# nz0001na/MorphGANformer

Measured on AMD Instinct MI355X. Metric: latent-projection iters/sec @1024^2, k=17 latents, higher is better.
Workload: dtype f32; 1 GPU; configs[1]: single 1024x1024 face per GPU, Wing+LPIPS(squeeze)+MSE literal-mode projection step, noise_mode=random, seeded synthetic weights/targets/landmarks; k=17, z_dim=32, targets_per_gpu=1, parallelism=pair-sharded x1, graph_replay=True, loss_generator_overlap=True, steps_per_forward=32

## Files before the change

include/mgf.h:

```cpp
#ifndef MGF_H_
#define MGF_H_

#include <stdint.h>

#ifdef __cplusplus
extern "C" {
#endif

typedef void* mgf_stream_t;

enum { MGF_OK = 0, MGF_EINVAL = -1, MGF_EUNSUPPORTED = -2, MGF_ELAUNCH = -3, MGF_ETOOBIG = -4 };
enum { MGF_F32 = 0, MGF_F64 = 1, MGF_F16 = 2 };
enum { MGF_FILTER_SEPARABLE = 2 };
enum { MGF_FILTER_LARGE = 4 };
enum { MGF_ACT_LINEAR = 1, MGF_ACT_RELU = 2, MGF_ACT_LRELU = 3, MGF_ACT_TANH = 4, MGF_ACT_SIGMOID = 5,
       MGF_ACT_ELU = 6, MGF_ACT_SELU = 7, MGF_ACT_SOFTPLUS = 8, MGF_ACT_SWISH = 9,
       MGF_ACT_RELU_POST = 10 };

const char* mgf_last_error(void);
int mgf_version(void);
int mgf_device_ok(void);

int mgf_bias_act(void* y, const void* x, const void* b, const void* xref, const void* yref, const void* dy,
                 int dtype, int64_t numel, int64_t step_b, int64_t size_b,
// ... 66 lines not shown
                                  const float* rgb_w, const float* rgb_bias, int32_t n, int32_t cin, int32_t h, int32_t w, int32_t cout,
                                  int32_t out_scale_stride, int32_t rgb_channels, mgf_stream_t stream);
int mgf_conv3x3_winograd2_f32(float* y, const float* x, const float* u, const float* in_scale, const float* out_scale, int32_t n,
                              int32_t cin, int32_t h, int32_t w, int32_t cout, int32_t out_scale_stride, const mgf_epilogue* ep,
                              mgf_stream_t stream);
int mgf_conv3x3_winograd3_f32(float* y, const float* x, const float* u, const float* in_scale, const float* out_scale, int32_t n,
                              int32_t cin, int32_t h, int32_t w, int32_t cout, int32_t out_scale_stride, const mgf_epilogue* ep,
                              mgf_stream_t stream);
int mgf_conv3x3_winograd3_slice_f32(float* y, const float* x, const float* u, const float* in_scale, const float* out_scale, int32_t n,
                                    int32_t cin, int32_t h, int32_t w, int32_t cout, int32_t out_scale_stride, int64_t y_batch,
                                    int32_t y_choff, const mgf_epilogue* ep, mgf_stream_t stream);
int mgf_conv1x1_f32(float* y, const float* x, const float* w, const float* in_scale, int32_t n, int32_t cin, int32_t hw, int32_t cout,
                    int32_t cout_pad, int64_t y_batch, int32_t y_choff, const mgf_epilogue* ep, mgf_stream_t stream);
int mgf_conv1x1_force_shape(int32_t channel_blocks);

int mgf_conv3x3s2_few_inputs_f32(float* y, const float* x, const float* w, const float* bias, int32_t n, int32_t cin, int32_t in_h,
                                 int32_t in_w, int32_t cout, int32_t relu, mgf_stream_t stream);
int mgf_tconv3x3s2_few_outputs_f32(float* y, const float* x, const float* wp, int32_t n, int32_t cin, int32_t h, int32_t w, int32_t cout,
                                   int32_t cout_pad, int32_t pitch, int64_t y_plane, int64_t y_batch, mgf_stream_t stream);
int mgf_conv3x3_winograd3_up2res_f32(float* y, const float* x, const float* u, const float* in_scale, const float* out_scale,
                                     const float* residual_low, int32_t n, int32_t cin, int32_t h, int32_t w, int32_t cout,
                                     int32_t out_scale_stride, const mgf_epilogue* ep, mgf_stream_t stream);
int mgf_winograd3_force_shape(int32_t shape);
int mgf_conv3x3_winograd3_rgb_f32(float* rgb_out, const float* x, const float* u, const float* in_scale, const float* out_scale,
                                  const float* rgb_w, const float* rgb_bias, int32_t n, int32_t cin, int32_t h, int32_t w, int32_t cout,
                                  int32_t out_scale_stride, int32_t rgb_channels, mgf_stream_t stream);
int mgf_conv3x3_winograd_f32(float* y, const float* x, const float* u, const float* in_scale, const float* out_scale, int32_t n,
                             int32_t cin, int32_t h, int32_t w, int32_t cout, int32_t out_scale_stride, const mgf_epilogue* ep,
                             mgf_stream_t stream);

int mgf_tconv3x3s2_border_f32(float* t, const float* x, const float* wp, const float* in_scale, const float* out_scale, int32_t n,
                              int32_t cin, int32_t h, int32_t w, int32_t cout, int32_t cout_pad, int64_t t_pitch, int64_t t_plane,
                              int64_t t_batch, int64_t out_scale_stride, mgf_stream_t stream);

int mgf_pack_conv_weights(float* wp, float* wsq, const float* w, int32_t cout, int32_t cin, int32_t kh, int32_t kw,
                          int32_t cout_pad, float gain, int32_t flip, mgf_stream_t stream);

typedef struct mgf_style_job {
    const float* aff_w;
    const float* aff_b;
    const float* wsq;
    float* s;
    float* d;
    int32_t cin, cout;
    int32_t w_offset;
    float aff_gain, style_gain;
} mgf_style_job;
int mgf_demod_f32(float* d, const float* s, const float* wsq, int32_t n, int32_t cin, int32_t cout, mgf_stream_t stream);
int mgf_demod_bwd_f32(float* ds, const float* dd, const float* d, const float* s, const float* wsq, int32_t n, int32_t cin, int32_t cout,
                      mgf_stream_t stream);
int mgf_style_demod(const mgf_style_job* job, const float* ws, int64_t ws_stride_n, int32_t n, int32_t wdim, mgf_stream_t stream);
int mgf_style_demod_multi(const mgf_style_job* jobs_dev, int32_t njobs, const float* ws, int64_t ws_stride_n,
                          int32_t n, int32_t wdim, int32_t max_cin, mgf_stream_t stream);

int mgf_duplex_attention(float* y, const float* x, const float* wqc, const float* spos, const float* vwb,
                         int32_t n, int32_t c, int32_t f, int32_t t,
                         const mgf_epilogue* ep, int32_t ep_w, float* probs, int32_t* argmax, mgf_stream_t stream);

int mgf_att_map_upsample_f32(float* out, const float* probs, int32_t n, int32_t side, int32_t t, int32_t out_res, int32_t layer,
                             int32_t n_layers, mgf_stream_t stream);

typedef struct mgf_attn_job {
    const float* wmv;
    const float* bmv;
    float* vwb;
    int32_t c;
// ... 188 lines not shown
```

morphganformer_amd/_lib.py:

```python
from __future__ import annotations

import ctypes as C
import os

import torch

HERE = os.path.dirname(os.path.abspath(__file__))
LIB_PATH = os.environ.get("MGF_LIB_PATH") or os.path.join(HERE, "libmgf_hip.so")

MGF_F32, MGF_F64, MGF_F16 = 0, 1, 2
ACT_IDS = {"linear": 1, "relu": 2, "lrelu": 3, "tanh": 4, "sigmoid": 5, "elu": 6, "selu": 7, "softplus": 8, "swish": 9,
           "relu_post": 10}
MAX_TAPS = 9

i32, i64, f32, f64, vp = C.c_int32, C.c_int64, C.c_float, C.c_double, C.c_void_p


class Epilogue(C.Structure):
    _fields_ = [("bias", vp), ("noise", vp), ("noise_strength", vp), ("noise_n", i32), ("act", i32), ("alpha", f32),
                ("gain", f32), ("residual", vp)]


class ConvDesc(C.Structure):
    _fields_ = [("n", i32), ("cin", i32), ("in_h", i32), ("in_w", i32), ("cout", i32), ("cout_pad", i32),
# ... 11 lines not shown
class StyleJob(C.Structure):
    _fields_ = [("aff_w", vp), ("aff_b", vp), ("wsq", vp), ("s", vp), ("d", vp), ("cin", i32), ("cout", i32),
                ("w_offset", i32), ("aff_gain", f32), ("style_gain", f32)]


class AttnJob(C.Structure):
    _fields_ = [("wmv", vp), ("bmv", vp), ("vwb", vp), ("c", i32), ("w_offset", i32)]


class StyleBwdJob(C.Structure):
    _fields_ = [("aff_w", vp), ("wsq", vp), ("s", vp), ("d", vp), ("ds_part", vp), ("dc_part", vp), ("cin", i32), ("cout", i32),
                ("s_chunks", i32), ("d_chunks", i32), ("aff_gain", f32), ("style_gain", f32)]


class AttnGradJob(C.Structure):
    _fields_ = [("dg", vp), ("probs", vp), ("dc", vp), ("cpre", vp), ("part", vp), ("dvwb", vp), ("dc_part", vp), ("c", i32), ("f", i32),
                ("slices", i32), ("nchunk", i32), ("blk_grad", i32), ("blk_dot", i32), ("blk_red", i32), ("pad_", i32)]


class AttnBwdJob(C.Structure):
    _fields_ = [("wmv", vp), ("dvwb", vp), ("c", i32), ("pad_", i32)]


_SIGS = {
    "mgf_last_error": (C.c_char_p, []),
    "mgf_version": (C.c_int, []),
    "mgf_device_ok": (C.c_int, []),
    "mgf_bias_act": (C.c_int, [vp, vp, vp, vp, vp, vp, C.c_int, i64, i64, i64, C.c_int, C.c_int, f32, f32, f32, vp]),
    "mgf_upfirdn2d": (C.c_int, [vp, vp, vp, C.c_int, i32, i32, i32, i32, i64, i64, i64, i64, i32, i32, i64, i64, i64, i64,
                                i32, i32, i32, i32, i32, i32, i32, i32, i32, i32, i32, f32, C.POINTER(Epilogue), vp]),
    "mgf_conv_taps_f32": (C.c_int, [vp, vp, vp, vp, vp, C.POINTER(ConvDesc), C.POINTER(Epilogue), vp]),
    "mgf_conv_taps_bf16x3_f32": (C.c_int, [vp, vp, vp, vp, vp, C.POINTER(ConvDesc), C.POINTER(Epilogue), vp]),
    "mgf_tconv3x3s2_border_f32": (C.c_int, [vp, vp, vp, vp, vp, i32, i32, i32, i32, i32, i32, i64, i64, i64, i64, vp]),
    "mgf_winograd_weights_f32": (C.c_int, [vp, vp, i32, i32, f32, vp]),
    "mgf_conv3x3_winograd_f32": (C.c_int, [vp, vp, vp, vp, vp, i32, i32, i32, i32, i32, i32, C.POINTER(Epilogue), vp]),
    "mgf_winograd2_weights_f32": (C.c_int, [vp, vp, i32, i32, f32, vp]),
    "mgf_conv3x3_winograd2_f32": (C.c_int, [vp, vp, vp, vp, vp, i32, i32, i32, i32, i32, i32, C.POINTER(Epilogue), vp]),
    "mgf_conv3x3_winograd2_rgb_f32": (C.c_int, [vp, vp, vp, vp, vp, vp, vp, i32, i32, i32, i32, i32, i32, i32, vp]),
    "mgf_conv3x3_winograd3_f32": (C.c_int, [vp, vp, vp, vp, vp, i32, i32, i32, i32, i32, i32, C.POINTER(Epilogue), vp]),
    "mgf_conv1x1_f32": (C.c_int, [vp, vp, vp, vp, i32, i32, i32, i32, i32, i64, i32, C.POINTER(Epilogue), vp]),
    "mgf_conv3x3s2_few_inputs_f32": (C.c_int, [vp, vp, vp, vp, i32, i32, i32, i32, i32, i32, vp]),
    "mgf_tconv3x3s2_few_outputs_f32": (C.c_int, [vp, vp, vp, i32, i32, i32, i32, i32, i32, i32, i64, i64, vp]),
    "mgf_conv1x1_force_shape": (C.c_int, [i32]),
    "mgf_conv3x3_winograd3_slice_f32": (C.c_int, [vp, vp, vp, vp, vp, i32, i32, i32, i32, i32, i32, i64, i32, C.POINTER(Epilogue), vp]),
    "mgf_conv3x3_winograd3_up2res_f32": (C.c_int, [vp, vp, vp, vp, vp, vp, i32, i32, i32, i32, i32, i32, C.POINTER(Epilogue), vp]),
    "mgf_winograd3_force_shape": (C.c_int, [i32]),
    "mgf_conv3x3_winograd3_rgb_f32": (C.c_int, [vp, vp, vp, vp, vp, vp, vp, i32, i32, i32, i32, i32, i32, i32, vp]),
    "mgf_conv3x3_winograd2_slice_f32": (C.c_int, [vp, vp, vp, vp, vp, i32, i32, i32, i32, i32, i32, i64, i32, C.POINTER(Epilogue), vp]),
    "mgf_pack_conv_weights": (C.c_int, [vp, vp, vp, i32, i32, i32, i32, i32, f32, i32, vp]),
    "mgf_conv_profile_begin": (C.c_int, []),
    "mgf_conv_profile_end": (C.c_int, [C.POINTER(ConvProfRec), i32]),
    "mgf_demod_f32": (C.c_int, [vp, vp, vp, i32, i32, i32, vp]),
    "mgf_demod_bwd_f32": (C.c_int, [vp, vp, vp, vp, vp, i32, i32, i32, vp]),
    "mgf_style_demod": (C.c_int, [C.POINTER(StyleJob), vp, i64, i32, i32, vp]),
    "mgf_style_demod_multi": (C.c_int, [vp, i32, vp, i64, i32, i32, i32, vp]),
    "mgf_duplex_attention": (C.c_int, [vp, vp, vp, vp, vp, i32, i32, i32, i32, C.POINTER(Epilogue), i32, vp, vp, vp]),
    "mgf_att_map_upsample_f32": (C.c_int, [vp, vp, i32, i32, i32, i32, i32, i32, vp]),
    "mgf_attn_values": (C.c_int, [C.POINTER(AttnJob), vp, i64, i64, i32, i32, i32, vp]),
    "mgf_attn_values_multi": (C.c_int, [vp, i32, vp, i64, i64, i32, i32, i32, vp]),
    "mgf_randn_f32": (C.c_int, [vp, i64, C.c_uint64, vp, vp]),
    "mgf_rgb_weights_f32": (C.c_int, [vp, vp, vp, i32, i32, i32, vp]),
    "mgf_torgb_compose_weights_f32": (C.c_int, [vp, vp, vp, vp, vp, vp, i32, i32, i32, i32, vp]),
    "mgf_conv3x3_few_outputs_f32": (C.c_int, [vp, vp, vp, vp, i32, i32, i32, i32, i32, vp]),
    "mgf_mapping_param_floats": (i64, [i32, i32, i32]),
    "mgf_mapping_forward": (C.c_int, [vp, vp, vp, i32, i32, i32, i32, i32, vp]),
    "mgf_reduce_scratch_floats": (i64, []),
# ... 134 lines not shown
```

morphganformer_amd/build.py:

```python
from __future__ import annotations

import glob
import hashlib
import os
import subprocess
import sys

HERE = os.path.dirname(os.path.abspath(__file__))
ROOT = os.path.dirname(HERE)
CSRC = os.path.join(HERE, "csrc")
OBJ = os.path.join(CSRC, "_obj")
LIB = os.path.join(HERE, "libmgf_hip.so")
SOURCES = ["capi.cpp", "bias_act.hip", "upfirdn2d.hip", "conv_taps.hip", "latent_prep.hip", "attention.hip", "losses.hip", "lpips_stem.hip",
           "embed.hip", "backward.hip", "wino.hip", "wino3.hip", "pointwise.hip", "narrow_conv.hip", "warp.hip", "lbp.hip", "mdf.hip"]
HEADERS = [os.path.join(CSRC, "mgf_common.h"), os.path.join(ROOT, "include", "mgf.h")]
HIPCC = os.environ.get("HIPCC", "/opt/rocm/bin/hipcc")
FLAGS = ["--offload-arch=gfx950", "-O3", "-fPIC", "-std=c++17", "-ffp-contract=on", "-Wno-unused-result", "-x", "hip"]
LINK_FLAGS = ["--offload-arch=gfx950", "-shared", "-fPIC"]

_compiler_id = None


def compiler_id() -> str:
    global _compiler_id
    if _compiler_id is None:
        _compiler_id = subprocess.run([HIPCC, "--version"], stdout=subprocess.PIPE, stderr=subprocess.STDOUT, check=True).stdout.decode()
    return _compiler_id


def object_key(src_path: str, flags) -> str:
    h = hashlib.sha256()
    h.update(compiler_id().encode())
    h.update("\0".join(flags).encode())
    for p in [src_path] + HEADERS:
        with open(p, "rb") as f:
            h.update(b"\0" + os.path.basename(p).encode() + b"\0" + f.read())
    return h.hexdigest()[:16]


def _compile_all(obj_dir, flags_for, verbose, force, prune=True):
    os.makedirs(obj_dir, exist_ok=True)
    objs, todo = [], []
    for src in SOURCES:
        sp = os.path.join(CSRC, src)
        flags = flags_for(src)
        op = os.path.join(obj_dir, f"{src}.{object_key(sp, flags)}.o")
        objs.append(op)
# ... 95 lines not shown
```

morphganformer_amd/conv.py:

```python
from __future__ import annotations

import ctypes as C
import os
from dataclasses import dataclass

import torch

from . import _lib


def round_up(v: int, m: int) -> int:
    return (v + m - 1) // m * m


def profile_begin():
    _lib.check(_lib.lib().mgf_conv_profile_begin(), "conv_profile_begin")


def profile_end(max_recs=4096):
    recs = (_lib.ConvProfRec * max_recs)()
    n = _lib.lib().mgf_conv_profile_end(recs, max_recs)
    if n < 0:
        _lib.check(n, "conv_profile_end")
    return [(recs[i].kernel.decode(), recs[i].flops, recs[i].seconds, recs[i].ksplit, recs[i].bytes) for i in range(min(n, max_recs))]
# ... 341 lines not shown
    return round_up(2 * w + 1, align)


def conv3x3s2_few_inputs(x, w, bias=None, relu=False, out=None):
    _lib.require_gpu(x, w, bias, out)
    cout, cin = w.shape[:2]
    assert tuple(w.shape[2:]) == (3, 3) and cin <= 4 and w.is_contiguous() and w.dtype == torch.float32
    assert x.dtype == torch.float32 and x.is_contiguous() and x.shape[1] == cin
    n, _, h, wd = x.shape
    oh, ow = (h - 3) // 2 + 1, (wd - 3) // 2 + 1
    if out is None:
        out = torch.empty([n, cout, oh, ow], dtype=torch.float32, device=x.device)
    assert out.is_contiguous() and tuple(out.shape) == (n, cout, oh, ow)
    rc = _lib.lib().mgf_conv3x3s2_few_inputs_f32(out.data_ptr(), x.data_ptr(), w.data_ptr(), _lib.ptr(bias), n, cin, h, wd, cout, int(relu),
                                                 _lib.stream_ptr())
    _lib.check(rc, "conv3x3s2_few_inputs")
    return out


def conv3x3_few_outputs(x, w, bias=None, out=None):
    _lib.require_gpu(x, w, bias, out)
    n, cin, h, wd = x.shape
    cout = w.shape[1]
    assert x.dtype == torch.float32 and x.is_contiguous() and w.dtype == torch.float32 and w.is_contiguous()
    assert tuple(w.shape) == (n, cout, cin, 3, 3) and cout <= 4
    if out is None:
        out = torch.empty([n, cout, h, wd], dtype=torch.float32, device=x.device)
    assert out.is_contiguous() and tuple(out.shape) == (n, cout, h, wd)
    _lib.check(_lib.lib().mgf_conv3x3_few_outputs_f32(out.data_ptr(), x.data_ptr(), w.data_ptr(), _lib.ptr(bias), n, cin, h, wd, cout,
                                                      _lib.stream_ptr()), "conv3x3_few_outputs")
    return out


def tconv3x3s2_forward(x, pc: PackedConv, in_scale=None, out_scale=None, out=None, bf=None):
    _lib.require_gpu(x, pc.wp, in_scale, out_scale, out)
    assert pc.kh == 3 and pc.kw == 3 and x.dtype == torch.float32 and x.is_contiguous()
    n, cin, h, w = x.shape
    oh, ow = 2 * h + 1, 2 * w + 1
    if out is None:
        out = torch.empty([n, pc.cout, oh, tconv_pitch(w)], dtype=torch.float32, device=x.device)
    pitch = out.shape[3]
    assert out.is_contiguous() and tuple(out.shape) == (n, pc.cout, oh, pitch) and pitch >= ow and pitch % 4 == 0
    if NARROW_CONV and pc.cout <= 4 and in_scale is None and out_scale is None:
        rc = _lib.lib().mgf_tconv3x3s2_few_outputs_f32(out.data_ptr(), x.data_ptr(), pc.wp.data_ptr(), n, cin, h, w, pc.cout, pc.cout_pad,
                                                       pitch, oh * pitch, pc.cout * oh * pitch, _lib.stream_ptr())
        _lib.check(rc, "tconv3x3s2_few_outputs")
        return out[:, :, :, :ow]
    split = SPLIT_TCONV_BORDER and min(h, w) >= (TCONV_SPLIT_MIN if n >= 4 else max(TCONV_SPLIT_MIN, 128))
    use_bf = bf is not None and split and w % 32 == 0 and cin % 16 == 0
    os_stride = 0 if out_scale is None else out_scale.stride(0) if out_scale.ndim == 2 else 0
    d = _desc(n, cin, h, w, pc.cout, pc.cout_pad, h if split else h + 1, w if split else w + 1, 1, 2, TCONV_TAPS, TCONV_GROUPS,
              [0, 0, 1, 1], [0, 1, 0, 1], oh, ow, pitch, oh * pitch, pc.cout * oh * pitch, 0, os_stride)
    if use_bf:
        rc = _lib.lib().mgf_conv_taps_bf16x3_f32(out.data_ptr(), x.data_ptr(), bf.data_ptr(), _lib.ptr(in_scale), _lib.ptr(out_scale),
                                                 C.byref(d), None, _lib.stream_ptr())
    else:
        rc = _lib.lib().mgf_conv_taps_f32(out.data_ptr(), x.data_ptr(), pc.wp.data_ptr(), _lib.ptr(in_scale), _lib.ptr(out_scale),
                                          C.byref(d), None, _lib.stream_ptr())
    _lib.check(rc, "conv_taps(tconv)")
    if split:
        rc = _lib.lib().mgf_tconv3x3s2_border_f32(out.data_ptr(), x.data_ptr(), pc.wp.data_ptr(), _lib.ptr(in_scale), _lib.ptr(out_scale),
                                                  n, cin, h, w, pc.cout, pc.cout_pad, pitch, oh * pitch, pc.cout * oh * pitch, os_stride,
                                                  _lib.stream_ptr())
        _lib.check(rc, "tconv3x3s2_border")
    return out[:, :, :, :ow]


def upfirdn_into(y, x, f2d, up=1, pad=(0, 0, 0, 0), gain=1.0, flip=False, epilogue=None, separable=False, down=1):
    _lib.require_gpu(x, y, f2d)
    n, c, h, w = x.shape
    fh, fw = f2d.shape
    px0, px1, py0, py1 = pad
    oh = (h * up + py0 + py1 - fh + down) // down
    ow = (w * up + px0 + px1 - fw + down) // down
    assert tuple(y.shape) == (n, c, oh, ow), (tuple(y.shape), (n, c, oh, ow))
    sx, sy = x.stride(), y.stride()
    rc = _lib.lib().mgf_upfirdn2d(y.data_ptr(), x.data_ptr(), f2d.data_ptr(), _lib.MGF_F32, n, c, h, w, sx[0], sx[1], sx[2],
                                  sx[3], oh, ow, sy[0], sy[1], sy[2], sy[3], fh, fw, up, up, down, down, px0, px1, py0, py1,
                                  int(flip) | (2 if separable else 0) | 4,
# ... 5 lines not shown
```

morphganformer_amd/engine.py:

```python
from __future__ import annotations

import ctypes as C
import math
import os
from dataclasses import dataclass, field

import numpy as np
import torch

from . import _lib
from . import conv as cv
from .synth_weights import GeneratorConfig

SQRT2 = math.sqrt(2.0)
SQRT_HALF = math.sqrt(0.5)
USE_WINOGRAD = os.environ.get("MGF_WINOGRAD", "1") != "0"
WINOGRAD_MAX_RES = int(os.environ.get("MGF_WINOGRAD_MAX_RES", "1024"))
BF_DIRECT_MAX_RES = int(os.environ.get("MGF_BF_DIRECT_MAX_RES", "128"))


def pack_mapping_params(sd, cfg: GeneratorConfig) -> np.ndarray:
    D, T = cfg.w_dim, cfg.k - 1
    lr = cfg.mapping_lrmul
    n_res = cfg.mapping_layers // 2
    g64 = lambda k: np.asarray(sd[k], dtype=np.float64)
    out = []

    def fc(prefix, lrmul):
        w = g64(prefix + ".weight")
        return w * (lrmul / math.sqrt(w.shape[1])), g64(prefix + ".bias") * lrmul

    for i in range(n_res):
        for j in (0, 1):
            w, b = fc(f"mapping.global_mlp.l{i}.fc{j}", lr)
            out += [w, b]
    out += list(fc("mapping.global_mlp.out_layer", lr))
    pos = g64("pos")
    for i in range(n_res):
        p = f"mapping.mlp.sa{i}"
        wq, bq = fc(p + ".to_queries", 1.0)
        wfp, bfp = fc(p + ".from_pos_map", 1.0)
        wk, bk = fc(p + ".to_keys", 1.0)
        wtp, btp = fc(p + ".to_pos_map", 1.0)
        wv, bv = fc(p + ".to_values", 1.0)
        wm, bm = fc(p + ".modulation", 1.0)
        sc = 1.0 / math.sqrt(D)
        out += [wq * sc, (bq[None] + pos @ wfp.T + bfp[None]) * sc, wk, bk[None] + pos @ wtp.T + btp[None], wv, bv, wm, bm]
        for j in (0, 1):
            w, b = fc(f"mapping.mlp.l{i}.fc{j}", lr)
            out += [w, b]
    out += list(fc("mapping.mlp.out_layer", lr))
    blob = np.concatenate([np.asarray(a, dtype=np.float64).reshape(-1) for a in out]).astype(np.float32)
    expect = _lib.lib().mgf_mapping_param_floats(cfg.k, D, n_res)
    assert blob.size == expect, (blob.size, expect)
    return blob


@dataclass
class ConvLayerPlan:
    name: str
    res: int
    cin: int
    cout: int
    up: int
    slot: int
    kind: str
    pc: cv.PackedConv = None
    aff_w: torch.Tensor = None
    aff_b: torch.Tensor = None
    style_gain: float = 1.0
    demod: bool = True
    bias: torch.Tensor = None
    noise_const: torch.Tensor = None
    noise_strength: torch.Tensor = None
    act_gain: float = 1.0
    attn: "AttnPlan" = None
    w_raw: torch.Tensor = None
    w_gained: torch.Tensor = None
    wino_u: torch.Tensor = None
    pcb: torch.Tensor = None
    s_off: int = 0
    d_off: int = 0


@dataclass
class AttnPlan:
    c: int
    f: int
    wqc: torch.Tensor
    spos: torch.Tensor
    wmv: torch.Tensor
    bmv: torch.Tensor
    v_off: int = 0


class SynthesisPlan:

    def __init__(self, sd, cfg: GeneratorConfig, device="cuda", arith="f32"):
        _lib.lib()
        self.cfg = cfg
        self.arith = arith
        self.device = torch.device(device)
        dev = self.device
        f64 = lambda k: np.asarray(sd[k], dtype=np.float64)
        t32 = lambda a: torch.as_tensor(np.ascontiguousarray(a, dtype=np.float32), device=dev)
        D, T = cfg.w_dim, cfg.k - 1
        self.mapping_blob = t32(pack_mapping_params(sd, cfg))
        self.const = t32(f64("synthesis.b4.const"))
        self.fir = t32(f64(f"synthesis.b{cfg.block_resolutions[-1]}.resample_kernel"))
        self.fir_is_1331 = bool(np.allclose(f64(f"synthesis.b{cfg.block_resolutions[-1]}.resample_kernel"),
                                            np.outer([1, 3, 3, 1], [1, 3, 3, 1]) / 64.0, rtol=0, atol=1e-7))
        self.layers: list[ConvLayerPlan] = []
        self.skips = {}
        s_off = d_off = v_off = 0
        for (res, name, cin, cout, up, slot, att, has_nb) in cfg.layer_table():
            p = f"synthesis.b{res}.{name}"
            w = f64(p + ".weight")
            kind = "torgb" if name == "torgb" else ("tconv" if up == 2 else "conv3")
            lp = ConvLayerPlan(name=p, res=res, cin=cin, cout=cout, up=up, slot=slot, kind=kind)
            if kind == "torgb":
                lp.pc = cv.pack_weights(t32(w), gain=1.0, flip=False)
                lp.w_raw = t32(w.reshape(cout, cin))
                lp.style_gain = 1.0 / math.sqrt(cin)
                lp.demod = False
            else:
                wg = 1.0 / math.sqrt(cin * 9)
                lp.pc = cv.pack_weights(t32(w), gain=wg, flip=False, want_wsq=True)
                if kind == "conv3" and USE_WINOGRAD and cv.winograd_ok(cin, cout, res, res) and res <= WINOGRAD_MAX_RES:
                    lp.wino_u = cv.winograd_pack(t32(w), wg, res)
                if arith == "bf16x3" and cin % 16 == 0 and res // up >= 32:
                    lp.pcb = cv.pack_weights_bf16x3(lp.pc)
            lp.aff_w = t32(f64(p + ".affine.weight"))
            lp.aff_b = t32(f64(p + ".affine.bias"))
            if (p + ".biasAct.bias") in sd:
                lp.bias = t32(f64(p + ".biasAct.bias"))
            if (p + ".noise_strength") in sd:
                lp.noise_strength = t32(f64(p + ".noise_strength").reshape(1))
                lp.noise_const = t32(f64(p + ".noise_const"))
            lp.act_gain = SQRT2 * (SQRT_HALF if (name == "conv1" and res > 4) else 1.0)
            if att and (p + ".transformer.to_queries.weight") in sd:
                lp.attn = self._fold_attention(sd, p, cout, res, T, D, t32, f64)
                lp.attn.v_off = v_off
                v_off += cout * T
            if name == "conv_last" and lp.bias is None and lp.noise_strength is None and lp.attn is None and cfg.img_channels <= 4:
                lp.w_gained = t32(w / math.sqrt(cin * 9))
            lp.s_off, lp.d_off = s_off, d_off
            s_off += cin
            d_off += cout
            self.layers.append(lp)
        self.s_total, self.d_total, self.v_total = s_off, d_off, v_off
        for res in cfg.block_resolutions[1:]:
            w = f64(f"synthesis.b{res}.skip.weight")
            self.skips[res] = cv.pack_weights(t32(w), gain=SQRT_HALF / math.sqrt(w.shape[1]), flip=False)
        torch.cuda.synchronize(dev)

    @staticmethod
    def _fold_attention(sd, p, C_, res, T, D, t32, f64):
        tp = p + ".transformer"
        Fn = res * res
        wq = f64(tp + ".to_queries.weight") / math.sqrt(C_)
        bq = f64(tp + ".to_queries.bias")
        wfp = f64(tp + ".from_pos_map.weight") / math.sqrt(D)
# ... 404 lines not shown
    def _draw_noise(self, n):
        sizes = [(lp.name, lp.res) for lp in self.plan.layers if lp.noise_strength is not None]
        total = sum(r * r for _, r in sizes)
        if self.noise_rand is None or self.noise_rand.numel() != n * total:
            self.noise_rand = torch.empty(n * total, dtype=torch.float32, device=self.device)
        if not torch.cuda.is_current_stream_capturing():
            gen = torch.cuda.default_generators[self.device.index if self.device.index is not None else torch.cuda.current_device()]
            seed, off = int(gen.initial_seed()), int(gen.get_offset())
            if (seed, off) != self._noise_epoch:
                self.noise_seed = (seed ^ (off * 0x9E3779B97F4A7C15)) & 0xFFFFFFFFFFFFFFFF
                self.noise_state.zero_()
            gen.set_offset(off + 4)
            self._noise_epoch = (seed, off + 4)
        _lib.check(_lib.lib().mgf_randn_f32(self.noise_rand.data_ptr(), self.noise_rand.numel(), self.noise_seed, self.noise_state.data_ptr(),
                                            _lib.stream_ptr()), "randn")
        out, off = {}, 0
        for name, r in sizes:
            out[name] = self.noise_rand[off * n:(off + r * r) * n].view(n, r * r)
            off += r * r
        return out

    def _bf_direct(self, lp, n, residual_low):
        return (lp.pcb is not None and lp.kind == "conv3" and residual_low is None and 32 <= lp.res <= BF_DIRECT_MAX_RES
                and n * (lp.res // 8) * (lp.res // 32) * (lp.cout // 32) >= 512)

    def _layer(self, lp, x, B, key, noise_mode, noises, residual, residual_low=None):
        n = x.shape[0]
        noise, noise_n = self._noise_for(lp, noise_mode, noises)
        ep = _lib.make_epilogue(bias=lp.bias, noise=noise, noise_strength=lp.noise_strength if noise is not None else None,
                                noise_n=noise_n, act="lrelu", alpha=0.2, gain=lp.act_gain, residual=residual)
        has_att = lp.attn is not None
        s, d = self._s(lp), self._d(lp)
        if lp.kind == "tconv":
            t = cv.tconv3x3s2_forward(x, lp.pc, in_scale=s, out_scale=d, out=B["t"], bf=lp.pcb)
            y = cv.upfirdn_into(B[key], t, self.plan.fir, up=1, pad=(1, 1, 1, 1), gain=4.0, epilogue=None if has_att else ep,
                                separable=True)
        elif self._bf_direct(lp, n, residual_low):
            y = cv.conv_forward(x, lp.pc, pad=(1, 1), in_scale=s, out_scale=d, epilogue=None if has_att else ep, out=B[key], bf=lp.pcb)
        elif lp.wino_u is not None and cv.winograd_fills_chip(n, lp.cout, lp.res, lp.res):
            y = cv.winograd_forward(x, lp.wino_u, in_scale=s, out_scale=d, epilogue=None if has_att else ep, out=B[key],
                                    residual_low=residual_low)
        else:
            y = cv.conv_forward(x, lp.pc, pad=(1, 1), in_scale=s, out_scale=d, epilogue=None if has_att else ep, out=B[key])
        if self.taps is not None:
            self.taps[lp.name + ":conv"] = y
        if has_att:
            a = lp.attn
            out = B[key + "a"]
            probs = argmax = None
            if self.att_maps is not None:
                probs = torch.empty([n, a.f, self.cfg.k - 1], dtype=torch.float32, device=self.device)
                argmax = torch.empty([n, a.f], dtype=torch.int32, device=self.device)
                self.att_maps[lp.name] = (probs, argmax)
            rc = _lib.lib().mgf_duplex_attention(out.data_ptr(), y.data_ptr(), a.wqc.data_ptr(), a.spos.data_ptr(),
                                                 self._v(lp).data_ptr(), n, a.c, a.f, self.cfg.k - 1, C.byref(ep), lp.res,
                                                 _lib.ptr(probs), _lib.ptr(argmax), _lib.stream_ptr())
            _lib.check(rc, "duplex_attention")
            y = out
        return y

    def forward_workspace(self, z=None, c=None, ws=None, truncation_psi=1, truncation_cutoff=None, return_img=True, return_att=False,
                          return_ws=False, subnet=None, noise_mode="random", noises=None, fused_modconv=None, att_format="tensor", lean=False):
        lean = bool(lean) and self.taps is None and not return_att
        nb = (z if ws is None else ws)
        if nb is not None and (nb.shape[0], lean) != (self.n, self.lean):
            self._alloc(nb.shape[0], lean)
        return_tensor = False
# ... 36 lines not shown
```

Baseline: 764.5 iters/s.

## Add Winograd-style MFMA kernel for stride-2 transposed 3x3 convolution interior

Adds a new HIP kernel that computes the interior of the stride-2 transposed 3x3 convolution with a Winograd-like decomposition. It uses 25 pre-transformed weight planes and MFMA 32x32x2 f32 instructions, with double-buffered LDS staging of input chunks. Border pixels are still written by the existing border kernel. The path is used for tconv layers up to 256 resolution when the workgroup count clears a threshold, and aims to cut multiply work and raise matrix-core use. In exchange it adds extra weight storage and a second kernel launch per layer, and the output is gated by fairly strict shape and alignment checks.

```diff
diff --git a/include/mgf.h b/include/mgf.h
--- a/include/mgf.h
+++ b/include/mgf.h
@@ -122,6 +122,11 @@
 int mgf_tconv3x3s2_border_f32(float* t, const float* x, const float* wp, const float* in_scale, const float* out_scale, int32_t n,
                               int32_t cin, int32_t h, int32_t w, int32_t cout, int32_t cout_pad, int64_t t_pitch, int64_t t_plane,
                               int64_t t_batch, int64_t out_scale_stride, mgf_stream_t stream);
+
+int mgf_tconv3x3s2_winograd_f32(float* t, const float* x, const float* u, const float* in_scale, const float* out_scale, int32_t n,
+                                int32_t cin, int32_t h, int32_t w, int32_t cout, int32_t pitch, int64_t t_plane, int64_t t_batch,
+                                int64_t out_scale_stride, mgf_stream_t stream);
+int mgf_tconv_winograd_weights_f32(float* u, const float* w, int32_t cout, int32_t cin, double gain, mgf_stream_t stream);
 
 int mgf_pack_conv_weights(float* wp, float* wsq, const float* w, int32_t cout, int32_t cin, int32_t kh, int32_t kw,
                           int32_t cout_pad, float gain, int32_t flip, mgf_stream_t stream);
diff --git a/morphganformer_amd/_lib.py b/morphganformer_amd/_lib.py
--- a/morphganformer_amd/_lib.py
+++ b/morphganformer_amd/_lib.py
@@ -67,6 +67,8 @@
     "mgf_conv_taps_f32": (C.c_int, [vp, vp, vp, vp, vp, C.POINTER(ConvDesc), C.POINTER(Epilogue), vp]),
     "mgf_conv_taps_bf16x3_f32": (C.c_int, [vp, vp, vp, vp, vp, C.POINTER(ConvDesc), C.POINTER(Epilogue), vp]),
     "mgf_tconv3x3s2_border_f32": (C.c_int, [vp, vp, vp, vp, vp, i32, i32, i32, i32, i32, i32, i64, i64, i64, i64, vp]),
+    "mgf_tconv3x3s2_winograd_f32": (C.c_int, [vp, vp, vp, vp, vp, i32, i32, i32, i32, i32, i32, i64, i64, i64, vp]),
+    "mgf_tconv_winograd_weights_f32": (C.c_int, [vp, vp, i32, i32, C.c_double, vp]),
     "mgf_winograd_weights_f32": (C.c_int, [vp, vp, i32, i32, f32, vp]),
     "mgf_conv3x3_winograd_f32": (C.c_int, [vp, vp, vp, vp, vp, i32, i32, i32, i32, i32, i32, C.POINTER(Epilogue), vp]),
     "mgf_winograd2_weights_f32": (C.c_int, [vp, vp, i32, i32, f32, vp]),
diff --git a/morphganformer_amd/build.py b/morphganformer_amd/build.py
--- a/morphganformer_amd/build.py
+++ b/morphganformer_amd/build.py
@@ -12,7 +12,8 @@
 OBJ = os.path.join(CSRC, "_obj")
 LIB = os.path.join(HERE, "libmgf_hip.so")
 SOURCES = ["capi.cpp", "bias_act.hip", "upfirdn2d.hip", "conv_taps.hip", "latent_prep.hip", "attention.hip", "losses.hip", "lpips_stem.hip",
-           "embed.hip", "backward.hip", "wino.hip", "wino3.hip", "pointwise.hip", "narrow_conv.hip", "warp.hip", "lbp.hip", "mdf.hip"]
+           "embed.hip", "backward.hip", "wino.hip", "wino3.hip", "pointwise.hip", "narrow_conv.hip", "warp.hip", "lbp.hip", "mdf.hip",
+           "wino_tconv.hip"]
 HEADERS = [os.path.join(CSRC, "mgf_common.h"), os.path.join(ROOT, "include", "mgf.h")]
 HIPCC = os.environ.get("HIPCC", "/opt/rocm/bin/hipcc")
 FLAGS = ["--offload-arch=gfx950", "-O3", "-fPIC", "-std=c++17", "-ffp-contract=on", "-Wno-unused-result", "-x", "hip"]
diff --git a/morphganformer_amd/conv.py b/morphganformer_amd/conv.py
--- a/morphganformer_amd/conv.py
+++ b/morphganformer_amd/conv.py
@@ -397,8 +397,29 @@
     return out
 
 
-def tconv3x3s2_forward(x, pc: PackedConv, in_scale=None, out_scale=None, out=None, bf=None):
-    _lib.require_gpu(x, pc.wp, in_scale, out_scale, out)
+TCONV_WINO = os.environ.get("MGF_TCONV_WINO", "1") != "0"
+TCONV_WINO_MIN_WGS = 4096
+
+
+def tconv_winograd_weights(w: torch.Tensor, gain: float = 1.0) -> torch.Tensor:
+    _lib.require_gpu(w)
+    w = w.contiguous().float()
+    cout, cin, kh, kw = w.shape
+    assert (kh, kw) == (3, 3) and cin % 4 == 0
+    u = torch.empty([25, cin // 4, cout, 4], dtype=torch.float32, device=w.device)
+    _lib.check(_lib.lib().mgf_tconv_winograd_weights_f32(u.data_ptr(), w.data_ptr(), cout, cin, float(gain), _lib.stream_ptr()),
+               "tconv_winograd_weights")
+    return u
+
+
+def tconv_winograd_ok(n, cin, h, w, cout, out, bf=None) -> bool:
+    return bool(TCONV_WINO and SPLIT_TCONV_BORDER and bf is None and h % 2 == 0 and w % 2 == 0 and min(h, w) >= TCONV_SPLIT_MIN and cin % 4 == 0 and cout % 32 == 0
+                and out.shape[3] % 4 == 0 and out.data_ptr() % 16 == 0
+                and n * -(-h // 4) * -(-w // 32) * (cout // 32) >= TCONV_WINO_MIN_WGS)
+
+
+def tconv3x3s2_forward(x, pc: PackedConv, in_scale=None, out_scale=None, out=None, bf=None, wt=None):
+    _lib.require_gpu(x, pc.wp, in_scale, out_scale, out, wt)
     assert pc.kh == 3 and pc.kw == 3 and x.dtype == torch.float32 and x.is_contiguous()
     n, cin, h, w = x.shape
     oh, ow = 2 * h + 1, 2 * w + 1
@@ -410,6 +431,17 @@
         rc = _lib.lib().mgf_tconv3x3s2_few_outputs_f32(out.data_ptr(), x.data_ptr(), pc.wp.data_ptr(), n, cin, h, w, pc.cout, pc.cout_pad,
                                                        pitch, oh * pitch, pc.cout * oh * pitch, _lib.stream_ptr())
         _lib.check(rc, "tconv3x3s2_few_outputs")
+        return out[:, :, :, :ow]
+    if wt is not None and tconv_winograd_ok(n, cin, h, w, pc.cout, out, bf):
+        assert tuple(wt.shape) == (25, cin // 4, pc.cout, 4)
+        os_stride = 0 if out_scale is None else out_scale.stride(0) if out_scale.ndim == 2 else 0
+        rc = _lib.lib().mgf_tconv3x3s2_winograd_f32(out.data_ptr(), x.data_ptr(), wt.data_ptr(), _lib.ptr(in_scale), _lib.ptr(out_scale), n, cin, h,
+                                                    w, pc.cout, pitch, oh * pitch, pc.cout * oh * pitch, os_stride, _lib.stream_ptr())
+        _lib.check(rc, "tconv3x3s2_winograd")
+        rc = _lib.lib().mgf_tconv3x3s2_border_f32(out.data_ptr(), x.data_ptr(), pc.wp.data_ptr(), _lib.ptr(in_scale), _lib.ptr(out_scale),
+                                                  n, cin, h, w, pc.cout, pc.cout_pad, pitch, oh * pitch, pc.cout * oh * pitch, os_stride,
+                                                  _lib.stream_ptr())
+        _lib.check(rc, "tconv3x3s2_border")
         return out[:, :, :, :ow]
     split = SPLIT_TCONV_BORDER and min(h, w) >= (TCONV_SPLIT_MIN if n >= 4 else max(TCONV_SPLIT_MIN, 128))
     use_bf = bf is not None and split and w % 32 == 0 and cin % 16 == 0
diff --git a/morphganformer_amd/csrc/wino_tconv.hip b/morphganformer_amd/csrc/wino_tconv.hip
--- /dev/null
+++ b/morphganformer_amd/csrc/wino_tconv.hip
@@ -0,0 +1,333 @@
+#include "mgf_common.h"
+#include <algorithm>
+#include <type_traits>
+
+namespace {
+
+typedef float f32x16 __attribute__((ext_vector_type(16)));
+typedef float v2f __attribute__((ext_vector_type(2)));
+
+constexpr int WTCK = 4;
+constexpr int WTFW = 34;
+constexpr int WTFH = 5;
+constexpr int WTFP = WTFH * WTFW;
+constexpr int WTNP = 25;
+constexpr int WTXS = 14;
+__constant__ float wt_ones[WTCK] = {1.f, 1.f, 1.f, 1.f};
+
+struct WinoTParams {
+    float* t;
+    const float* x;
+    const float* u;
+    const float* in_scale;
+    const float* out_scale;
+    int n, cin, h, w, cout, os_stride, pitch;
+    int tiles_x, tiles_y, co_tiles;
+    int xcd_per;
+    int64_t t_plane, t_batch;
+};
+
+__global__ __launch_bounds__(256, 2) void wino_tconv_kernel(WinoTParams p) {
+    constexpr int CST = 256, RAW = WTCK * CST;
+    extern __shared__ float lds[];
+    float* const raw0 = lds;
+    float* const raw1 = raw0 + RAW;
+    const int tid = threadIdx.x, lane = tid & 63;
+    const int a = __builtin_amdgcn_readfirstlane(tid >> 6);
+    const int l31 = lane & 31, half = lane >> 5;
+    const int tx = l31 & 15, ty = l31 >> 4;
+
+    int b_ = blockIdx.x;
+    if (p.xcd_per > 0) {
+        b_ = (b_ & 7) * p.xcd_per + (b_ >> 3);
+        if (b_ >= p.n * p.tiles_x * p.tiles_y * p.co_tiles) return;
+    }
+    const int cot = b_ % p.co_tiles; b_ /= p.co_tiles;
+    const int ptx = b_ % p.tiles_x; b_ /= p.tiles_x;
+    const int pty = b_ % p.tiles_y;
+    const int n = b_ / p.tiles_y;
+    const int co0 = cot * 32, iy0 = pty * 4, ix0 = ptx * 32;
+    const int plane = p.h * p.w;
+    const float* xn = p.x + (int64_t)n * p.cin * plane;
+    const float* sc = p.in_scale ? p.in_scale + (int64_t)n * p.cin : nullptr;
+    const int nck = p.cin / WTCK;
+
+    const __amdgpu_buffer_rsrc_t rx = __builtin_amdgcn_make_buffer_rsrc((void*)xn, 0, p.cin * plane * 4, 0x00020000);
+    const __amdgpu_buffer_rsrc_t ru = __builtin_amdgcn_make_buffer_rsrc((void*)p.u, 0, WTNP * p.cin * p.cout * 4, 0x00020000);
+    const __amdgpu_buffer_rsrc_t rnull = __builtin_amdgcn_make_buffer_rsrc((void*)p.u, 0, 0, 0x00020000);
+    unsigned xoff;
+    {
+        const int r = tid / WTFW, q = tid - r * WTFW;
+        const int iy = iy0 - 1 + r, ix = ix0 - 1 + q;
+        xoff = (tid < WTFP && iy >= 0 && iy < p.h && ix >= 0 && ix < p.w) ? (unsigned)(iy * p.w + ix) * 4u : 0xFFFFFFF0u;
+    }
+    const unsigned aoff = (unsigned)(((co0 + l31) * WTCK + half * 2) * 4);
+    const int upos = nck * p.cout * WTCK * 4;
+    const int ubase_row = 5 * a * upos, ubase_col = (20 + a) * upos, ubase_sh = 24 * upos + (a & 1) * 4;
+
+    float xr[WTCK];
+    auto load_x = [&](float (&dst)[WTCK], int c0, bool live = true) {
+        const __amdgpu_buffer_rsrc_t r = live ? rx : rnull;
+#pragma unroll
+        for (int j = 0; j < WTCK; ++j) dst[j] = __builtin_bit_cast(float, __builtin_amdgcn_raw_buffer_load_b32(r, xoff, (c0 + j) * plane * 4, 0));
+    };
+    typedef const float __attribute__((address_space(4)))* cfp4;
+    const cfp4 sbase = sc ? (cfp4)sc : (cfp4)wt_ones;
+    const int sstep = sc ? 1 : 0;
+    auto load_s = [&](float (&dst)[WTCK], int c0) {
+#pragma unroll
+        for (int j = 0; j < WTCK; ++j) dst[j] = sbase[c0 * sstep + j];
+    };
+    auto park_x = [&](float* R, const float (&src)[WTCK], const float (&sv)[WTCK]) {
+#pragma unroll
+        for (int j = 0; j < WTCK; ++j) R[j * CST + tid] = src[j] * sv[j];
+    };
+    struct Aop { v2f q[6]; float s; };
+    auto load_a = [&](Aop& dst, int c0, bool live = true) {
+        const int soff = c0 * p.cout * 4;
+        const __amdgpu_buffer_rsrc_t r = live ? ru : rnull;
+#pragma unroll
+        for (int b = 0; b < 5; ++b)
+            dst.q[b] = __builtin_bit_cast(v2f, __builtin_amdgcn_raw_buffer_load_b64(r, aoff, ubase_row + b * upos + soff, 0));
+        dst.q[5] = __builtin_bit_cast(v2f, __builtin_amdgcn_raw_buffer_load_b64(r, aoff, ubase_col + soff, 0));
+        dst.s = __builtin_bit_cast(float, __builtin_amdgcn_raw_buffer_load_b32(r, aoff, ubase_sh + soff, 0));
+    };
+    const int pr = a == 0 ? 0 : (a == 2 ? 2 : 1);
+    const float sg = (a == 0 || a == 2) ? -1.f : 0.f;
+    const int px = a == 0 ? 0 : (a == 2 ? 2 : 1);
+    const float sgf = (a == 0 || a == 2) ? -1.f : 0.f;
+    auto transform = [&](float (&B)[2][6], const float* R) {
+#pragma unroll
+        for (int kk = 0; kk < 2; ++kk) {
+            const float* src = R + (half + 2 * kk) * CST + 2 * ty * WTFW + 2 * tx;
+            const float* rp = src + pr * WTFW;
+            const float* r1 = src + WTFW;
+            const float* r2 = src + 2 * WTFW;
+            const v2f p01 = *reinterpret_cast<const v2f*>(rp), q01 = *reinterpret_cast<const v2f*>(r1), f01 = *reinterpret_cast<const v2f*>(r2);
+            const float p2 = rp[2], q2 = r1[2], f2 = r2[2];
+            const v2f sg2 = {sg, sg};
+            const v2f e01 = p01 + sg2 * q01;
+            const float e2 = p2 + sg * q2;
+            B[kk][0] = e01.x - e01.y;
+            B[kk][1] = e01.y;
+            B[kk][2] = e2 - e01.y;
+            B[kk][3] = e2;
+            const float fp = px == 0 ? f01.x : (px == 2 ? f2 : f01.y);
+            B[kk][4] = fp + sgf * f01.y;
+            B[kk][5] = f2;
+        }
+    };
+
+    f32x16 acc[6];
+    f32x16 accs = {};
+    constexpr int BI[5] = {0, 1, 2, 1, 3};
+    auto mfma_chunk = [&](const Aop& A, const float (&B)[2][6], auto first_tag, auto parity_tag) {
+        constexpr bool FIRST = decltype(first_tag)::value;
+        constexpr int PAR = decltype(parity_tag)::value;
+#pragma unroll
+        for (int b = 0; b < 6; ++b) {
+            const int bi = b < 5 ? BI[b] : 4;
+            acc[b] = __builtin_amdgcn_mfma_f32_32x32x2f32(A.q[b].x, B[0][bi], FIRST ? f32x16{} : acc[b], 0, 0, 0);
+            acc[b] = __builtin_amdgcn_mfma_f32_32x32x2f32(A.q[b].y, B[1][bi], acc[b], 0, 0, 0);
+        }
+        if ((a >> 1) == PAR) {
+            const float bs = (a & 1) ? B[1][5] : B[0][5];
+            accs = __builtin_amdgcn_mfma_f32_32x32x2f32(A.s, bs, accs, 0, 0, 0);
+        }
+    };
+
+    const int nchunks = nck;
+    const int last = nchunks - 1;
+    auto chunk0 = [&](int i) { return (i < last ? i : last) * WTCK; };
+    Aop A0, A1;
+    float B0[2][6], B1[2][6];
+    float sv[WTCK];
+    {
+        float xa[WTCK], xb[WTCK], sa_[WTCK], sb_[WTCK];
+        load_s(sv, chunk0(2));
+        load_x(xa, 0);
+        load_a(A0, 0);
+        load_x(xb, chunk0(1));
+        load_x(xr, chunk0(2));
+        load_s(sa_, 0);
+        load_s(sb_, chunk0(1));
+        park_x(raw0, xa, sa_);
+        park_x(raw1, xb, sb_);
+        __syncthreads();
+        transform(B0, raw0);
+        __syncthreads();
+    }
+    auto body = [&](int i, Aop& Acur, Aop& Anxt, float (&Bcur)[2][6], float (&Bnxt)[2][6], float* raw_nxt, float* raw_park, auto first_tag,
+                    auto parity_tag) {
+        load_a(Anxt, chunk0(i + 1), i + 1 < nchunks);
+        __builtin_amdgcn_sched_barrier(0);
+        transform(Bnxt, raw_nxt);
+        mfma_chunk(Acur, Bcur, first_tag, parity_tag);
+        __builtin_amdgcn_sched_barrier(0);
+        park_x(raw_park, xr, sv);
+        load_x(xr, chunk0(i + 3), i + 3 < nchunks);
+        load_s(sv, chunk0(i + 3));
+        __syncthreads();
+    };
+    using P0 = std::integral_constant<int, 0>;
+    using P1 = std::integral_constant<int, 1>;
+    body(0, A0, A1, B0, B1, raw1, raw0, std::true_type{}, P0{});
+    if (1 < nchunks) body(1, A1, A0, B1, B0, raw0, raw1, std::false_type{}, P1{});
+    for (int it = 2; it < nchunks; it += 2) {
+        body(it, A0, A1, B0, B1, raw1, raw0, std::false_type{}, P0{});
+        if (it + 1 < nchunks) body(it + 1, A1, A0, B1, B0, raw0, raw1, std::false_type{}, P1{});
+    }
+
+    float R[4][16];
+#pragma unroll
+    for (int v = 0; v < 16; ++v) {
+        R[0][v] = acc[0][v] + acc[1][v];
+        R[1][v] = acc[3][v];
+        R[2][v] = acc[1][v] + acc[2][v];
+        R[3][v] = acc[4][v];
+    }
+    float* const xch = lds;
+    auto put = [&](int slot, const float* vals) {
+        float* dst = xch + slot * 1024 + lane;
+#pragma unroll
+        for (int v = 0; v < 16; ++v) dst[v * 64] = vals[v];
+    };
+    float colv[16], shv[16];
+#pragma unroll
+    for (int v = 0; v < 16; ++v) { colv[v] = acc[5][v]; shv[v] = accs[v]; }
+    if (a == 1) {
+#pragma unroll
+        for (int j = 0; j < 4; ++j) put(j, R[j]);
+        put(10, colv);
+        put(11, shv);
+    } else if (a == 2) {
+#pragma unroll
+        for (int j = 0; j < 4; ++j) put(4 + j, R[j]);
+    } else if (a == 0) {
+        put(8, colv);
+        put(9, shv);
+    } else {
+        put(12, colv);
+        put(13, shv);
+    }
+    __syncthreads();
+    const float* xl = xch + lane;
+    float Y[4][16];
+    if (a == 0 || a == 1) {
+        const int s0 = a == 0 ? 0 : 4;
+#pragma unroll
+        for (int j = 0; j < 4; ++j)
+#pragma unroll
+            for (int v = 0; v < 16; ++v) Y[j][v] = R[j][v] + xl[(s0 + j) * 1024 + v * 64];
+    } else if (a == 2) {
+#pragma unroll
+        for (int v = 0; v < 16; ++v) {
+            const float m51 = xl[8 * 1024 + v * 64], m52 = xl[10 * 1024 + v * 64], m54 = xl[12 * 1024 + v * 64];
+            Y[0][v] = m51 + m52;
+            Y[1][v] = m54;
+            Y[2][v] = m52 + colv[v];
+            Y[3][v] = (xl[9 * 1024 + v * 64] + xl[11 * 1024 + v * 64]) + (shv[v] + xl[13 * 1024 + v * 64]);
+        }
+    } else {
+#pragma unroll
+        for (int j = 0; j < 4; ++j)
+#pragma unroll
+            for (int v = 0; v < 16; ++v) Y[j][v] = R[j][v];
+    }
+    const int orow = a == 0 ? 0 : (a == 1 ? 2 : (a == 2 ? 3 : 1));
+    const int by = iy0 + 2 * ty, bx = ix0 + 2 * tx;
+    const bool ok = by < p.h && bx < p.w;
+    const int cob = co0 + 4 * half;
+    const float* osc = p.out_scale ? p.out_scale + (int64_t)n * p.os_stride + cob : nullptr;
+    const unsigned toff = ok ? (unsigned)(((int64_t)cob * p.t_plane + (int64_t)(2 * by + orow) * p.pitch + 2 * bx) * 4) : 0xFFFFFFF0u;
+    typedef unsigned v4u __attribute__((ext_vector_type(4)));
+    const __amdgpu_buffer_rsrc_t rt = __builtin_amdgcn_make_buffer_rsrc((void*)(p.t + (int64_t)n * p.t_batch), 0,
+                                                                       (int)((int64_t)p.cout * p.t_plane * 4), 0x00020000);
+#pragma unroll
+    for (int v = 0; v < 16; ++v) {
+        const int cl = (v & 3) + 8 * (v >> 2);
+        const float s = osc ? osc[cl] : 1.f;
+        const v4u o = {__builtin_bit_cast(unsigned, Y[0][v] * s), __builtin_bit_cast(unsigned, Y[1][v] * s),
+                       __builtin_bit_cast(unsigned, Y[2][v] * s), __builtin_bit_cast(unsigned, Y[3][v] * s)};
+        __builtin_amdgcn_raw_buffer_store_b128(o, rt, toff, (int)(cl * p.t_plane * 4), 0);
+    }
+}
+
+__global__ __launch_bounds__(256) void wino_tconv_weights_kernel(float* u, const float* w, int cout, int cin, double gain) {
+    const int64_t total = (int64_t)cout * cin;
+    for (int64_t i = (int64_t)blockIdx.x * 256 + threadIdx.x; i < total; i += (int64_t)gridDim.x * 256) {
+        const int co = (int)(i % cout), ci = (int)(i / cout);
+        const float* g = w + ((int64_t)co * cin + ci) * 9;
+        double t[5][3];
+#pragma unroll
+        for (int v = 0; v < 3; ++v) {
+            const double g0 = g[v], g1 = g[3 + v], g2 = g[6 + v];
+            t[0][v] = g2;
+            t[1][v] = g0 + g2;
+            t[2][v] = g0;
+            t[3][v] = g1;
+            t[4][v] = g1;
+        }
+        const int cl = ci & 3, slot = 2 * (cl & 1) + (cl >> 1);
+        const int64_t pl = (int64_t)cin * cout;
+        float* dst = u + (((int64_t)(ci >> 2)) * cout + co) * 4 + slot;
+#pragma unroll
+        for (int r = 0; r < 5; ++r) {
+            const double o[5] = {t[r][2], t[r][0] + t[r][2], t[r][0], t[r][1], t[r][1]};
+#pragma unroll
+            for (int c = 0; c < 5; ++c) dst[(5 * r + c) * pl] = (float)(o[c] * gain);
+        }
+    }
+}
+
+}
+
+extern "C" int mgf_tconv_winograd_weights_f32(float* u, const float* w, int32_t cout, int32_t cin, double gain, mgf_stream_t stream) {
+    MGF_REQUIRE(u && w && cout >= 1 && cin >= 1, MGF_EINVAL, "tconv_winograd_weights: bad arguments");
+    MGF_REQUIRE(cin % WTCK == 0, MGF_EUNSUPPORTED, "tconv_winograd_weights: cin must be a multiple of %d (got %d)", WTCK, cin);
+    hipLaunchKernelGGL(wino_tconv_weights_kernel, dim3(mgf_stream_grid((int64_t)cout * cin, 256, 1)), dim3(256), 0, (hipStream_t)stream, u, w, cout,
+                       cin, gain);
+    MGF_CHECK_LAUNCH("tconv_winograd_weights");
+    return MGF_OK;
+}
+
+extern "C" int mgf_tconv3x3s2_winograd_f32(float* t, const float* x, const float* u, const float* in_scale, const float* out_scale, int32_t n,
+                                           int32_t cin, int32_t h, int32_t w, int32_t cout, int32_t pitch, int64_t t_plane, int64_t t_batch,
+                                           int64_t out_scale_stride, mgf_stream_t stream) {
+    MGF_REQUIRE(t && x && u && n >= 1 && cin >= 1 && cout >= 1 && h >= 2 && w >= 2, MGF_EINVAL, "tconv3x3s2_winograd: bad arguments");
+    MGF_REQUIRE(cin % WTCK == 0 && cout % 32 == 0, MGF_EUNSUPPORTED, "tconv3x3s2_winograd: cin must be a multiple of %d and cout of 32 (got %d, %d)",
+                WTCK, cin, cout);
+    MGF_REQUIRE(h % 2 == 0 && w % 2 == 0, MGF_EUNSUPPORTED, "tconv3x3s2_winograd: even map sides only (got %dx%d)", h, w);
+    MGF_REQUIRE(pitch >= 2 * w + 1 && pitch % 4 == 0 && t_plane >= (int64_t)(2 * h + 1) * pitch && t_plane % 4 == 0 && t_batch % 4 == 0 &&
+                    t_batch >= (int64_t)cout * t_plane, MGF_EINVAL, "tconv3x3s2_winograd: bad workspace layout");
+    MGF_REQUIRE(((uintptr_t)t % 16) == 0 && ((uintptr_t)u % 16) == 0, MGF_EINVAL, "tconv3x3s2_winograd: t and u must be 16-byte aligned");
+    MGF_REQUIRE((int64_t)cin * h * w <= INT32_MAX / 4 && (int64_t)WTNP * cin * cout <= INT32_MAX / 4 && (int64_t)cout * t_plane <= INT32_MAX / 4,
+                MGF_ETOOBIG, "tconv3x3s2_winograd: one sample / the weight planes must stay below 2 GiB (32-bit buffer offsets)");
+    WinoTParams p{};
+    p.t = t; p.x = x; p.u = u; p.in_scale = in_scale; p.out_scale = out_scale;
+    p.n = n; p.cin = cin; p.h = h; p.w = w; p.cout = cout; p.os_stride = (int)out_scale_stride; p.pitch = pitch;
+    p.t_plane = t_plane; p.t_batch = t_batch;
+    p.tiles_x = (int)mgf_cdiv(w, 32);
+    p.tiles_y = (int)mgf_cdiv(h, 4);
+    p.co_tiles = cout / 32;
+    int64_t blocks = (int64_t)n * p.tiles_x * p.tiles_y * p.co_tiles;
+    MGF_REQUIRE(blocks <= INT32_MAX - 8, MGF_ETOOBIG, "tconv3x3s2_winograd: too many workgroups");
+    p.xcd_per = 0;
+    if ((int64_t)WTNP * cin * cout * 4 <= (4 << 20) && blocks >= 16) {
+        p.xcd_per = (int)((blocks + 7) / 8);
+        blocks = (int64_t)p.xcd_per * 8;
+    }
+    const size_t lds = std::max<size_t>((size_t)2 * WTCK * 256, (size_t)WTXS * 16 * 64) * sizeof(float);
+    static bool attr_set = false;
+    if (!attr_set) {
+        hipError_t e = hipFuncSetAttribute((const void*)wino_tconv_kernel, hipFuncAttributeMaxDynamicSharedMemorySize, 65536);
+        if (e != hipSuccess) { mgf_set_error("tconv3x3s2_winograd: cannot raise dynamic LDS: %s", hipGetErrorString(e)); return MGF_ELAUNCH; }
+        attr_set = true;
+    }
+    mgf_prof_external_begin((hipStream_t)stream, "wino_tconv_kernel", 2.0 * 9 * cin * (double)cout * h * w * n,
+                            4.0 * ((double)n * cin * h * w + 9.0 * cin * cout + (double)n * cout * 4.0 * h * w));
+    hipLaunchKernelGGL(wino_tconv_kernel, dim3((unsigned)blocks), dim3(256), lds, (hipStream_t)stream, p);
+    mgf_prof_external_end((hipStream_t)stream);
+    MGF_CHECK_LAUNCH("tconv3x3s2_winograd");
+    return MGF_OK;
+}
diff --git a/morphganformer_amd/engine.py b/morphganformer_amd/engine.py
--- a/morphganformer_amd/engine.py
+++ b/morphganformer_amd/engine.py
@@ -16,6 +16,7 @@
 SQRT_HALF = math.sqrt(0.5)
 USE_WINOGRAD = os.environ.get("MGF_WINOGRAD", "1") != "0"
 WINOGRAD_MAX_RES = int(os.environ.get("MGF_WINOGRAD_MAX_RES", "1024"))
+TCONV_WINO_MAX_RES = int(os.environ.get("MGF_TCONV_WINO_MAX_RES", "256"))
 BF_DIRECT_MAX_RES = int(os.environ.get("MGF_BF_DIRECT_MAX_RES", "128"))
 
 
@@ -78,6 +79,7 @@
     w_raw: torch.Tensor = None
     w_gained: torch.Tensor = None
     wino_u: torch.Tensor = None
+    wino_t: torch.Tensor = None
     pcb: torch.Tensor = None
     s_off: int = 0
     d_off: int = 0
@@ -128,6 +130,9 @@
                 lp.pc = cv.pack_weights(t32(w), gain=wg, flip=False, want_wsq=True)
                 if kind == "conv3" and USE_WINOGRAD and cv.winograd_ok(cin, cout, res, res) and res <= WINOGRAD_MAX_RES:
                     lp.wino_u = cv.winograd_pack(t32(w), wg, res)
+                if (kind == "tconv" and arith != "bf16x3" and cv.TCONV_WINO and res <= TCONV_WINO_MAX_RES and cin % 4 == 0
+                        and cout % 32 == 0):
+                    lp.wino_t = cv.tconv_winograd_weights(t32(w), wg)
                 if arith == "bf16x3" and cin % 16 == 0 and res // up >= 32:
                     lp.pcb = cv.pack_weights_bf16x3(lp.pc)
             lp.aff_w = t32(f64(p + ".affine.weight"))
@@ -598,7 +603,7 @@
         has_att = lp.attn is not None
         s, d = self._s(lp), self._d(lp)
         if lp.kind == "tconv":
-            t = cv.tconv3x3s2_forward(x, lp.pc, in_scale=s, out_scale=d, out=B["t"], bf=lp.pcb)
+            t = cv.tconv3x3s2_forward(x, lp.pc, in_scale=s, out_scale=d, out=B["t"], bf=lp.pcb, wt=lp.wino_t)
             y = cv.upfirdn_into(B[key], t, self.plan.fir, up=1, pad=(1, 1, 1, 1), gain=4.0, epilogue=None if has_att else ep,
                                 separable=True)
         elif self._bf_direct(lp, n, residual_low):
```

Measured after the change: 779.1 iters/s (median of 6 runs). 1.9% higher.
